# scraed/LanPaint

Measured on AMD Instinct MI355X. Metric: langevin_think_iterations_per_sec, higher is better.
Workload: dtype f32; 1 GPU; c2_sdxl: latent 1x4x128x128 per GPU, 30 sigmas x 5 think iterations, 50% box mask, stub backbone x->(0.9x,0.8x), VE/Karras schedule; rng=torch, graph=auto, mask_format=f32, mask_seen_by_kernels=bits, captured_calls=1, backbone_io=f32, replicas=1, rows_per_gpu=1, global_rows=1, latent_elements_per_gpu=65536

## Files before the change

include/lanpaint_hip.h:

```cpp
#ifndef LANPAINT_HIP_H
#define LANPAINT_HIP_H

#include <stdint.h>

#ifdef __cplusplus
extern "C" {
#endif

#define LP_ABI_VERSION 25

#define LP_API __attribute__((visibility("default")))

#define LP_OK             0
#define LP_E_INVALID     -1
#define LP_E_UNSUPPORTED -2
#define LP_E_LAUNCH      -3
#define LP_E_ALIGN       -4

#define LP_COEF_STRIDE   36
#define LP_C_SCALE        0
#define LP_C_SQRT_ABT     1
#define LP_C_OMA          2
#define LP_C_ABT          3
#define LP_C_RSIGMA       4
// ... 41 lines not shown
#define LP_FL_MASK_U8       (1u << 2)
#define LP_FL_WRITE_X0S     (1u << 3)
#define LP_FL_X0_BF16       (1u << 4)
#define LP_FL_X0_F16        (1u << 5)
#define LP_FL_XIN_BF16      (1u << 6)
#define LP_FL_XIN_F16       (1u << 7)
#define LP_FL_PER_ELEMENT   (1u << 8)
#define LP_FL_CFG_FUSED     (1u << 10)
#define LP_FL_MASK_BITS     (1u << 11)
#define LP_FL_NO_REGION_SKIP (1u << 12)
#define LP_FL_ES            (1u << 13)
#define LP_FL_ES_GATED      (1u << 14)
#define LP_FL_ES_CLOSE      (1u << 15)
#define LP_FL_ES_RING_BITS  (1u << 16)
#define LP_FL_AV            (1u << 17)
#define LP_FL_X0S_GIVEN     (1u << 9)

typedef struct lp_es_state {
    int32_t  stopped;
    int32_t  counter;
    int32_t  n_ran;
    int32_t  cur_slot;
    int32_t  anchor_slot;
    int32_t  write_slot;
    uint32_t reserved0;
    int32_t  enabled;
    int64_t  seq_base;
    int64_t  total_ran;
    double   threshold_eff;
    double   abt_val;
// ... 888 lines not shown
```

lanpaint_amd/_cabi.py:

```python
from __future__ import annotations

import ctypes as C
import os

_HERE = os.path.dirname(os.path.abspath(__file__))
LIB_NAME = "liblanpaint_hip.so"
LIB_PATH = os.path.join(_HERE, LIB_NAME)
ABI_VERSION = 25

LP_OK, LP_E_INVALID, LP_E_UNSUPPORTED, LP_E_LAUNCH, LP_E_ALIGN = 0, -1, -2, -3, -4
LP_COEF_STRIDE = 36
(LP_C_SCALE, LP_C_SQRT_ABT, LP_C_OMA, LP_C_ABT, LP_C_RSIGMA, LP_C_DTX, LP_C_DTY, LP_C_AX, LP_C_AY, LP_C_DX, LP_C_DY,
 LP_C_VALID) = range(12)
LP_C_REGION0, LP_C_REGION1, LP_C_TMODEL, LP_C_RSCALE = 12, 22, 32, 33
(LP_R_E_FULL, LP_R_K_FULL, LP_R_STD_FULL, LP_R_E_HALF, LP_R_K_HALF, LP_R_STD_HALF, LP_R_DT, LP_R_A, LP_R_CX0,
 LP_R_CXT) = range(10)

LP_PH_REPLACE, LP_PH_POST_FIRST, LP_PH_POST_STEADY, LP_PH_PRE_HALF, LP_PH_EMIT, LP_PH_COEFFS, LP_PH_SIGMA = 1, 2, 4, 8, 16, 32, 64
LP_FL_FLOW, LP_FL_MASK_DENOISE, LP_FL_MASK_U8, LP_FL_WRITE_X0S = 1, 2, 4, 8
LP_FL_X0_BF16, LP_FL_X0_F16, LP_FL_XIN_BF16, LP_FL_XIN_F16 = 16, 32, 64, 128
LP_FL_PER_ELEMENT, LP_FL_X0S_GIVEN, LP_FL_CFG_FUSED, LP_FL_MASK_BITS, LP_FL_NO_REGION_SKIP = 256, 512, 1024, 2048, 4096
LP_FL_ES, LP_FL_ES_GATED, LP_FL_ES_CLOSE, LP_FL_ES_RING_BITS, LP_FL_AV = 1 << 13, 1 << 14, 1 << 15, 1 << 16, 1 << 17
LP_TUNE_VEC1, LP_TUNE_VEC4, LP_TUNE_ES_NO_DECIDE, LP_TUNE_ES_NO_FOLD, LP_TUNE_ES_NO_ATOMICS = 1, 2, 4, 8, 16


def mask_bits_bytes(n_el: int) -> int:
    return ((int(n_el) + 63) // 64) * 8
LP_REPLACE_KNOWN, LP_REPLACE_VE, LP_REPLACE_FLOW = 0, 1, 2
LP_RNG_PHILOX, LP_RNG_TORCH = 0, 1
LP_NN_ATEN_SCALAR, LP_NN_ATEN_CPU_GENERIC_FMA, LP_NN_ATEN_CPU_GENERIC = 0, 1, 2
LP_RESHAPE_BINARIZE, LP_RESHAPE_RULE_SHIFT = 1, 8


class LpHyper(C.Structure):
    _fields_ = [("lambda_", C.c_float), ("beta", C.c_float), ("step_size", C.c_float), ("min_step_frac", C.c_float),
                ("is_flow", C.c_int32), ("one_plus_lambda", C.c_float)]

# ... 637 lines not shown
```

lanpaint_amd/buffers.py:

```python
from __future__ import annotations

import weakref

import torch

from . import _cabi
from ._util import tensor_version

class _Workspace:

    def __init__(self, like: torch.Tensor, static_io: bool = False, model_dtype=None):
        self.shape, self.device = tuple(like.shape), like.device
        self.x_t = torch.empty_like(like)
        self.C = torch.empty_like(like)
        self.coef = torch.empty((like.shape[0], _cabi.LP_COEF_STRIDE), dtype=torch.float32, device=like.device)
        self.coef_av = None
        self.av_times = None
        self.x0s = []
        self.static_io = static_io
        if static_io:
            self.x_final = torch.empty_like(like)
            self.x_in = self.x_final if model_dtype is None else torch.empty_like(like, dtype=model_dtype)

    def matches(self, like):
# ... 58 lines not shown
        return self.ring[3] if self.ring is not None else None

    def wait(self, seq, device):
        i64 = self.i64
        for _ in range(20000):
            if i64[0] >= seq:
                return
        torch.cuda.current_stream(device).synchronize()
        if i64[0] < seq:
            raise RuntimeError("early-stop mailbox was not written (expected sequence %d, found %d)" % (seq, int(i64[0])))


class _CallState:
    __slots__ = ("input_x", "xc", "shape", "n_el", "rows", "flow", "ws", "stream", "sigma", "y", "m", "m_c", "m_flag", "abt",
                 "current_times", "base_flags", "keep", "t_model", "sigma_model", "compat", "n_steps", "x_final", "x_in",
                 "xin_flag", "k0_desc", "replace_kind_static", "out", "es")


class _CapturedCall:

    def __init__(self, counter):
        self.graph = torch.cuda.CUDAGraph()
        self.counter = counter
        self.ws = None
        self.final = None
        self.ran = 0
        self.launches = 0
        self.keep = None
        self.fast = False
        self.rows, self.flow, self.hyper, self.k0_desc, self.f_desc = 0, False, None, None, None
        self.call = None
        self.raw_exec = None
        self.ident = None
        self.final_in_graph = False
        self.es = None
        self.n_steps = 0
        self.key = None
        self.tail = None
        self.model_options = None
        self.alive = True
        self.siblings = {}
        self.times_seen = ()
        self.node_table = None
        self.binding = None
        self.tail_handles = None
        self.sigma_root = None

    def __del__(self):
        sr, self.sigma_root = self.sigma_root, None
# ... 12 lines not shown
```

lanpaint_amd/capture.py:

```python
from __future__ import annotations

import ctypes
import os
import weakref

import torch

from . import _cabi
from ._util import _gc_hold, _gc_release
from .buffers import _CapturedCall, _Workspace
from .masks import _compact_mask


class GraphReplay:

    MAX_GRAPHS = 16
    AUTO_MAX_BACKBONE_HOST_US = 100.0

    def begin_call(self, x, latent_image, noise, sigma, latent_mask, current_times, model_options, seed):
        cap = self._last_cap
        if cap is None or cap.tail is None or self.model_dtype is not None or not x.is_cuda:
            return None
        self.img_dim_size = len(x.shape)
        self.latent_image, self.noise = latent_image, noise
# ... 174 lines not shown
        for seen in cap.times_seen:
            if seen[0] is ve and seen[1] is abt and seen[2] is ft:
                return True
        ok = (i[13] == ve.numel() and i[14] == abt.numel() and i[15] == ft.numel() and ve.dtype == f32 and abt.dtype == f32
              and ft.dtype == f32 and ve.is_contiguous() and abt.is_contiguous() and ft.is_contiguous())
        if ok:
            cap.times_seen = (cap.times_seen + ((ve, abt, ft),))[-2:]
        return ok

    def _hyper_key(self):
        return (self.chara_lamb, self.chara_beta, self.step_size, self.min_step_frac)

    def _override_state(self):
        d, t, o = self.__dict__, type(self), self._OWN_METHODS
        return ("langevin_dynamics" in d or t.langevin_dynamics is not o[0], "score_model" in d or t.score_model is not o[1],
                "prepare_step_size" in d or t.prepare_step_size is not o[2], self.IS_FLUX, self.IS_FLOW, self.model_dtype)

    def _graph_eligible(self, x, model_options, sigma, current_times):
        if not self.graph or self._graph_blocked or callable(self.rng) or self._noise_regenerated:
            return False
        rows = x.shape[0] if x.ndim else 1
        if any(t.numel() not in (1, rows) for t in (sigma, *current_times)):
            return False
        if self.audio_indicator is not None or self.audio_correction is not None:
            if (self.audio_indicator is None or self.current_times_audio is None
                    or any(t.numel() not in (1, rows) for t in self.current_times_audio)
                    or os.environ.get("LANPAINT_AMD_AV_TABLE", "1") == "0"):
                return False
            packed = self._indicator_pack(self.audio_indicator, x.shape)
            if packed is None or (self._es_opts is not None and not packed[2]):
                return False
# ... 50 lines not shown
            out_b = self.LanPaint(xb, sigma, latent_mask, current_times, n_steps, model_options, seed, IS_FLUX, IS_FLOW)
            same = bool(torch.equal(out_a, out_b)) and bool(torch.equal(xa, xb))
        except Exception as e:
            return give_up("checking the capture against eager launches failed (%s)" % type(e).__name__)
        if not same:
            return give_up("a replayed sigma call does not reproduce the eager one (the backbone keeps state the graph does not see)")
        self._iterations_run, _, _, self._torch_consumed, self._philox_offset = saved
        torch.cuda.set_rng_state(saved[1], dev)
        return cap

    def _call_graphed(self, x, sigma, latent_mask, current_times, n_steps, model_options, seed, IS_FLUX, IS_FLOW):
        m_c, _ = _compact_mask(latent_mask, x.shape, x.device)
        key = (tuple(x.shape), x.device.index, int(n_steps), bool(IS_FLUX), bool(IS_FLOW), self.latent_image.data_ptr(),
               latent_mask.data_ptr(), m_c.data_ptr() if m_c is not None else 0, int(sigma.numel()),
               tuple(int(t.numel()) for t in current_times), id(model_options), seed, self.rng, self._hyper_key(),
               self.model_dtype, None if self._es_opts is None else (self._es_opts["threshold"], self._es_opts["patience_eff"],
                                                                      self._es_opts["trace"] is not None),
               None if self.audio_indicator is None else (self._indicator_pack(self.audio_indicator, x.shape)[0].data_ptr(),
                                                          self.audio_correction is not None))
        cap = self._graphs.get(key)
        if cap is not None and cap.model_options is not model_options:
            del self._graphs[key]
            cap.alive = False
            cap = None
        if cap is None:
            capture = self._auto_capture if self.graph == "auto" else self._capture
            cap = capture(key, x, sigma, latent_mask, current_times, n_steps, model_options, seed, IS_FLUX, IS_FLOW)
            if cap is None:
                return self.LanPaint(x, sigma, latent_mask, current_times, n_steps, model_options, seed, IS_FLUX, IS_FLOW)
            while len(self._graphs) > self.MAX_GRAPHS:
                self._graphs.popitem(last=False)[1].alive = False
# ... 9 lines not shown
            self._last_cap = None
            return self.LanPaint(x, sigma, latent_mask, current_times, n_steps, model_options, seed, IS_FLUX, IS_FLOW)
        self._iterations_run += cap.ran
        self.last_inner_steps = cap.ran
        if fast:
            if not isinstance(model_options, dict) or "lanpaint_semantic_stop" not in model_options:
                cap.ident = (self.latent_image, latent_mask, model_options, x.shape, n_steps, seed, self.rng,
                             self.latent_image.data_ptr(), latent_mask.data_ptr(), getattr(latent_mask, "_lp_bits", None),
                             getattr(latent_mask, "_lp_u8", None), x.device, sigma.numel(), current_times[0].numel(),
                             current_times[1].numel(), current_times[2].numel(), self._override_state(), self._hyper_key())
                self._last_cap = cap
            return self._replay_fast(cap, x, sigma, current_times)
        self._last_cap = None
        st = self._prologue(x, sigma, latent_mask, current_times, n_steps, model_options, seed, IS_FLUX, IS_FLOW, ws=cap.ws,
                            ds=cap.es["ds"] if cap.es is not None else None)
        cap.graph.replay()
        if self.rng == "torch":
            gen = self._generator(x.device)
            gen.set_offset(gen.get_offset() + cap.launches)
            self._torch_consumed += cap.launches
        out = self._epilogue(st, cap.final, rng_bump=(cap.counter, cap.launches) if self.rng == "philox" else None,
                             in_graph=cap.final_in_graph)
        if cap.es is not None and st.es is not None:
            self._es_after_replay(cap, st.es["seq"], x.device)
        return out

    def _replay_fast(self, cap, x, sigma, current_times):
        lib, stream = self._lib, self._stream(x.device)
        ve, abt = current_times[0], current_times[1]
        t_src = current_times[2] if cap.flow else ve
        out = torch.empty_like(x)
        k0, f = cap.k0_desc, cap.f_desc
        k0.x, k0.noise = x.data_ptr(), self.noise.data_ptr()
        k0.t_ve, k0.t_abt, k0.t_rsig, k0.t_model = ve.data_ptr(), abt.data_ptr(), sigma.data_ptr(), t_src.data_ptr()
        if cap.final_in_graph:
            k0.io_table_val[0], k0.io_table_val[1] = k0.x, out.data_ptr()
        else:
            f.x_dst, f.out = k0.x, out.data_ptr()
        if self.rng == "torch":
            gen = self._generator(x.device)
            off = gen.get_offset()
            k0.rng_state_val[0], k0.rng_state_val[1] = off, gen.initial_seed()
            gen.set_offset(off + cap.launches)
            self._torch_consumed += cap.launches
        seq = 0
        if cap.es is not None:
            seq = k0.es_seq_base = cap.es["ds"].next_seq()
        if cap.raw_exec is not None:
            _cabi.check(lib.lp_replay_call(ctypes.byref(cap.call), stream), "lp_replay_call")
        else:
            _cabi.check(lib.lp_step(ctypes.byref(k0), stream), "lp_step")
# ... 118 lines not shown
                    cap.final_in_graph = True
        finally:
            self._capturing = None
            _gc_release()
        cap.launches = self._cap_offset
        self._es_opts = es_user
        torch.cuda.set_rng_state(rng_state, dev)
        cap.ran = self._iterations_run - it0
        self._iterations_run = it0
        cap.keep = st
        cap.rows, cap.flow = st.rows, st.flow
        cap.hyper = _cabi.LpHyper.from_buffer_copy(self._hyper)
        cap.k0_desc = st.k0_desc
        cap.f_desc = f
        cap.model_options = model_options
        cap.es, cap.n_steps = st.es, st.n_steps
        cap.fast = bool(dense_ok and st.k0_desc is not None and st.replace_kind_static and st.xc is st.input_x)
        if replace_in_graph:
            ok = cap.fast and cap.final_in_graph
            if ok:
                try:
                    cap.graph.instantiate()
                    raw_graph = int(cap.graph.raw_cuda_graph())
                    cap.raw_exec = int(cap.graph.raw_cuda_graph_exec()) or None
                    b = _cabi.LpGraphBinding()
                    ok = cap.raw_exec is not None and self._lib.lp_graph_bind_replace(
                        raw_graph, ctypes.byref(cap.k0_desc), ctypes.byref(b)) == _cabi.LP_OK
                    if ok:
                        cap.binding = b
                        tg, te = ctypes.c_void_p(), ctypes.c_void_p()
                        if self._lib.lp_graph_clone_tail(raw_graph, ctypes.byref(tg), ctypes.byref(te)) == _cabi.LP_OK:
# ... 28 lines not shown
```

lanpaint_amd/csrc/aux_kernels.hip:

```cpp
#include "lp_common.h"

namespace lp {

__global__ void lp_coeffs_kernel(lp_hyper h, const float* __restrict__ ve, int ve_stride,
                                 const float* __restrict__ abt, int abt_stride, const float* __restrict__ rs,
                                 int rs_stride, const float* __restrict__ step_ov, int step_stride,
                                 const float* __restrict__ t_model, int t_stride, int rows, float* __restrict__ table) {
    const int t = blockIdx.x * blockDim.x + threadIdx.x;
    const int r = t >> 2;
    if (r >= rows) return;
    const float abt_f = abt[static_cast<int64_t>(r) * abt_stride];
    const float ve_f = ve ? ve[static_cast<int64_t>(r) * ve_stride] : 0.0f;
    const float rs_f = rs ? rs[static_cast<int64_t>(r) * rs_stride] : 0.0f;
    const float tm_f = t_model ? t_model[static_cast<int64_t>(r) * t_stride] : 0.0f;
    const float oma = 1.0f - abt_f;
    const float step = step_ov ? step_ov[static_cast<int64_t>(r) * step_stride]
                               : h.step_size * fmaxf(oma, h.min_step_frac);
    coeffs_lane(h, abt_f, ve_f, rs_f, tm_f, step, (t >> 1) & 1, t & 1, table + static_cast<int64_t>(r) * LP_COEF_STRIDE);
}

__global__ void lp_sigma_times_kernel(const float* __restrict__ sigma, int rows, const float* __restrict__ schedule,
                                      int schedule_len, int is_flow, float* __restrict__ times,
                                      float* __restrict__ scalars, int32_t* __restrict__ seq_out, int32_t seq,
                                      const SigmaRule rule) {
// ... 26 lines not shown
    hipLaunchKernelGGL(lp_coeffs_kernel, dim3((lanes + block - 1) / block), dim3(block), 0, stream, *h, ve, ve_stride,
                       abt, abt_stride, rs, rs_stride, step_ov, step_stride, t_model, t_stride, rows, table);
    return hipGetLastError() == hipSuccess ? LP_OK : LP_E_LAUNCH;
}

template <int VEC, int BLOCK>
__global__ __launch_bounds__(256) void lp_finalize_kernel(const void* a_mask, const void* a_model_out, const float* a_y,
                                                          const float* a_x_src, const uint64_t* a_io_table, int64_t a_n_el,
                                                          uint32_t a_flags, const lp_final_desc d_arg) {
    lp_final_desc d = d_arg;
    d.mask = a_mask; d.model_out = a_model_out; d.y = a_y; d.x_src = a_x_src; d.io_table = a_io_table;
    d.n_el = a_n_el; d.flags = a_flags;
    const int64_t groups = d.n_el / VEC;
    const int dt = x0_dtype(d.flags);
    const int64_t g = static_cast<int64_t>(blockIdx.x) * BLOCK + threadIdx.x;
    float* const x_dst = d.io_table ? reinterpret_cast<float*>(d.io_table[0]) : d.x_dst;
    float* const out = d.io_table ? reinterpret_cast<float*>(d.io_table[1]) : d.out;
    if (d.io_table && d.io_table[2] == 0ull) return;
    constexpr bool RA = VEC == 4 && BLOCK == 256;
    const bool in_range = g < groups;
    if (RA || in_range) {
        const int64_t i = (in_range ? g : groups - 1) * VEC;
        float m[VEC], mo[VEC], yv[VEC], o[VEC];
        Raw<VEC> m_raw, mo_raw, un_raw;
        load_mask_raw<VEC>(d.mask, d.flags, i, m_raw);
        float xs[VEC];
        bool need_mo = true, need_y = true;
        if constexpr (RA) {
            if (x_dst) load_f32<VEC>(d.x_src, i, xs);
            if ((d.flags & LP_FL_MASK_BITS) && !(d.flags & (LP_FL_CFG_FUSED | LP_FL_NO_REGION_SKIP))) {
                const uint32_t nib = (m_raw.w[0] >> (static_cast<uint32_t>(i) & 31u)) & 0xFu;
// ... 20 lines not shown
        }
#pragma unroll
        for (int k = 0; k < VEC; ++k) o[k] = mo[k] * (1.0f - m[k]) + yv[k] * m[k];
        store_f32<VEC>(out, i, o);
        if (x_dst) store_f32<VEC>(x_dst, i, xs);
    }
    if (d.rng_bump_ptr && blockIdx.x == 0 && threadIdx.x == 0) *d.rng_bump_ptr += d.rng_bump;
}

static bool aligned(const void* p, size_t a) { return p == nullptr || (reinterpret_cast<uintptr_t>(p) % a) == 0; }

int finalize_dispatch(const lp_final_desc* dp, hipStream_t stream) {
    if (!dp) return LP_E_INVALID;
    const lp_final_desc& d = *dp;
    if (d.n_el <= 0 || !d.model_out || !d.y || !d.mask || (!d.out && !d.io_table)) return LP_E_INVALID;
    if ((d.x_dst || d.io_table) && !d.x_src) return LP_E_INVALID;
    if ((d.flags & LP_FL_CFG_FUSED) && !d.uncond) return LP_E_INVALID;
    if ((d.flags & LP_FL_MASK_BITS) && ((d.flags & (LP_FL_MASK_U8 | LP_FL_MASK_DENOISE)) || !aligned(d.mask, 4)))
        return LP_E_INVALID;
    const bool half = x0_dtype(d.flags) != DT_F32;
    const bool vec4 = (d.n_el % 4 == 0) && aligned(d.model_out, half ? 8 : 16) && aligned(d.uncond, half ? 8 : 16) &&
                      aligned(d.y, 16) &&
                      aligned(d.mask, (d.flags & (LP_FL_MASK_U8 | LP_FL_MASK_BITS)) ? 4 : 16) && aligned(d.x_src, 16) &&
                      (d.io_table ? true : (aligned(d.x_dst, 16) && aligned(d.out, 16)));
    const int vec = vec4 ? 4 : 1;
    const int64_t groups = d.n_el / vec;
    const int block = groups <= 64 * 1024 ? 64 : 256;
    const int64_t bx = (groups + block - 1) / block;
    if (bx > 0x7fffffff) return LP_E_INVALID;
#define LP_FINAL_ARGS d.mask, d.model_out, d.y, d.x_src, d.io_table, d.n_el, d.flags, d
    const dim3 grid(static_cast<unsigned>(bx));
// ... 239 lines not shown
```

lanpaint_amd/csrc/step_kernel.hip:

```cpp
#include <cstddef>

#include "lp_common.h"

#pragma clang fp contract(off)

namespace lp {

struct RegionCoef {
    float e_full, k_full, std_full, e_half, k_half, std_half, dt, a, cx0, cxt;
};

struct RowCoef {
    float scale, sqrt_abt, oma, abt, rsigma, dtx, dty, ax, ay, dx, dy, valid;
    RegionCoef reg[2];
    float rscale;
};

__device__ __forceinline__ RowCoef load_row(const float* __restrict__ coef, int row) {
    const float* c = coef + static_cast<int64_t>(row) * LP_COEF_STRIDE;
    RowCoef r;
    r.scale = c[LP_C_SCALE]; r.sqrt_abt = c[LP_C_SQRT_ABT]; r.oma = c[LP_C_OMA]; r.abt = c[LP_C_ABT];
    r.rsigma = c[LP_C_RSIGMA]; r.dtx = c[LP_C_DTX]; r.dty = c[LP_C_DTY]; r.ax = c[LP_C_AX]; r.ay = c[LP_C_AY];
    r.dx = c[LP_C_DX]; r.dy = c[LP_C_DY]; r.valid = c[LP_C_VALID];
    r.rscale = c[LP_C_RSCALE];
// ... 296 lines not shown
        row = static_cast<int>(st_base / epr) + static_cast<int>(blockIdx.y - st_round * per_round);
        const int64_t row_lo = static_cast<int64_t>(row) * epr, row_hi = row_lo + epr;
        st_lo = row_lo > st_base ? row_lo : st_base;
        st_hi = row_hi < st_base + span ? row_hi : st_base + span;
        if (row >= d.rows || st_lo >= st_hi) return;
        const int64_t i0 = st_base + static_cast<int64_t>(blockIdx.x) * kBlock, i1 = i0 + kBlock;
        bool any = false;
#pragma unroll
        for (int k = 0; k < 4; ++k) {
            const int64_t s0 = i0 + k * static_cast<int64_t>(d.rng_bg), s1 = i1 + k * static_cast<int64_t>(d.rng_bg);
            any = any || (s0 < st_hi && s1 > st_lo);
        }
        if (!any) return;
    }
    const uint32_t fl = d.flags;
    bool es_gated = false, es_idle = false;
    int es_prev = -1, es_anchor = -1, es_write = 0;
    bool es_keeper = false;
    lp_es_state es_lite;
    uint2 es_words[8];
    double es_fv[kEsSums];
    if constexpr (ES) {
        es_gated = (fl & LP_FL_ES_GATED) != 0;
        if constexpr (es_fold) {
            const int rd = (d.es_index + 1) & 1;
            const lp_es_state* sp = d.es + rd;
            if constexpr (VEC == 4) {
                const uint2* sv = reinterpret_cast<const uint2*>(sp);
#pragma unroll
                for (int k = 0; k < 8; ++k) es_words[k] = sv[k];
// ... 346 lines not shown
        if (post) {
            if constexpr (PAIR) {
                if (need_x0) load_raw_pair(d.x0, i, pair_x0, x0_raw);
                if (!(d.x0_big == d.x0 || given) && need_known) load_raw_pair(d.x0_big, i, pair_known, x0b_raw);
            } else {
                if (need_x0 && lane_x0) load_raw_w<VEC, X0W>(d.x0, x0dt, i_x0, x0_raw);
                if (!(d.x0_big == d.x0 || given) && need_known && lane_known) load_raw_w<VEC, X0W>(d.x0_big, x0dt, i_kn, x0b_raw);
            }
        }
        if constexpr (TS) {
            asm volatile("" ::"s"(rng_w0), "s"(rng_w1), "s"(d.rng_offset), "s"(d.rng_seed), "s"(d.rng_inc),
                         "s"(reinterpret_cast<uintptr_t>(d.mask)), "s"(reinterpret_cast<uintptr_t>(d.y)),
                         "s"(reinterpret_cast<uintptr_t>(d.x_in)), "s"(reinterpret_cast<uintptr_t>(d.x0s)),
                         "s"(HARD ? uintptr_t(0) : reinterpret_cast<uintptr_t>(d.corr_el)), "s"(d.lambda),
                         "s"(d.one_plus_lambda), "s"(d.cfg_scale), "s"(d.cfg_scale_big));
        }
        if constexpr (SMALL) load_mask_raw<VEC>(d.mask, mfl, i, m_raw);
        const bool has_corr = (TS && HARD) ? false : (d.corr_el != nullptr && !given);
        const bool host_post = HOT ? false : d.xi_post != nullptr, host_pre = HOT ? false : d.xi_pre != nullptr;
        const bool need_rng = (post && !host_post) || ((ph & LP_PH_PRE_HALF) && !host_pre);
        if (post) {
            if (!given && need_known && lane_known) load_f32<VEC>(d.y, i_kn, yv);
            if (host_post) load_f32<VEC>(d.xi_post, i, xi_a);
            if (has_corr) load_f32<VEC>(d.corr_el, i, corr);
        }
        if ((ph & LP_PH_PRE_HALF) && host_pre) load_f32<VEC>(d.xi_pre, i, xi_b);
        float x0p[VEC], anc[VEC], rg[VEC], es_b0[VEC], es_b1[VEC], es_b2[VEC];
        constexpr bool RING_BITS_ONLY = ES != 0 && HARD && PH != 0;
        const bool ring_bits = RING_BITS_ONLY || (fl & LP_FL_ES_RING_BITS) != 0;
        uint32_t rg_raw = 0u;
// ... 27 lines not shown
                }
                if constexpr (!(es_fold && VEC == 4)) {
                    load_ring();
                }
            }
        }

        if constexpr (!SMALL) {
            if (need_rng && d.rng_offset_ptr) {
                rng_w0 = d.rng_offset_ptr[0];
                rng_w1 = d.rng_offset_ptr[1];
                rng_have = true;
            }
        }
        if constexpr (!TS) {
        if (d.io_table_out && el_bx == 0 && blockIdx.y == 0 && threadIdx.x == 0) {
            d.io_table_out[0] = d.io_table_val[0];
            d.io_table_out[1] = d.io_table_val[1];
            if (d.io_valid) d.io_table_out[2] = 1ull;
        }
        }
        if constexpr (PH == 0 || (PH & LP_PH_REPLACE) != 0) {
            if (d.es_reset && d.es && el_bx == 0 && blockIdx.y == 0) {
                if (d.es_partials) {
                    for (int k = threadIdx.x; k < kEsSets * kEsSlots * 8; k += kBlock) d.es_partials[k] = 0.0;
                }
                if (threadIdx.x == 0) es_reset_state(d, fold_coeffs);
            }
        }
        if constexpr (TBL) {
            float abt_f, ve_f, rs_f, tm_f;
// ... 67 lines not shown
                    }
                } else {
#pragma unroll
                for (int k = 0; k < VEC; ++k) {
                    float za, zb;
                    const uint64_t e = static_cast<uint64_t>(elem_index(i, k));
                    if (key_uniform) normal_pair_key<PH != 0>(static_cast<uint32_t>(e), static_cast<uint32_t>(seq), key0, za, zb);
                    else normal_pair(e, seq, seed, za, zb);
                    if (!host_post) xi_a[k] = za;
                    if (!host_pre) xi_b[k] = zb;
                }
                }
            }
        }

        if constexpr (TS) {
            __builtin_amdgcn_sched_barrier(0);
            if constexpr (X0W == 2) {
                uint16_t h = static_cast<uint16_t>(x0_raw.w[0]);
                asm volatile("" : "+v"(h) : "v"(xi_a[0]));
                x0_raw.w[0] = h;
            } else {
                asm volatile("" : "+v"(x0_raw.w[0]) : "v"(xi_a[0]));
            }
        }
        if constexpr (ES == 2 && VEC == 4) {
            if (post) {
                if (es_prev >= 0) load_f32<VEC>(es_prev == 0 ? d.es_x0s[0] : es_prev == 1 ? d.es_x0s[1] : d.es_x0s[2], i, x0p);
                load_ring();
            }
// ... 273 lines not shown
                for (int k = 0; k < VEC; ++k) {
                    const float ha = half_valid(xt[k], cv[k], xi_b[k], rc.reg[0]), hb = half_valid(xt[k], cv[k], xi_b[k], rc.reg[1]);
                    xe[k] = m[k] == 1.0f ? hb : ha;
                }
            } else {
#pragma unroll
                for (int k = 0; k < VEC; ++k) xe[k] = half_step(xt[k], cv[k], xi_b[k], k);
            }
            if (!(ES && es_gated)) {
#pragma unroll
                for (int k = 0; k < VEC; ++k) xt[k] = xe[k];
            }
        }

        LP_CLK(5)
        if (post && live) store_f32<VEC>(d.C, i, cv);
        if ((ph & kTouchXt) && live) store_f32<VEC>(d.x_t, i, xt);
        if constexpr (ES) {
            if (es_gated && (ph & LP_PH_PRE_HALF) && live) store_f32<VEC>(d.es_xte, i, xe);
            if (es_fold && es_idle) load_f32<VEC>(d.x_t, i, xe);
        }

        if (ph & LP_PH_EMIT) {
            float xo[VEC];
            if constexpr (VEC == 4 && !PER_EL && PH != 0) {
                const float sc = rc.scale;
                if (flow) {
                    float y;
                    if constexpr (ES != 0 || (RNG == 1 && !ST)) {
                        y = 1.0f / sc;
                        asm volatile("" : "+v"(y));
                    } else {
// ... 10 lines not shown
                for (int k = 0; k < VEC; ++k) {
                    float sc;
                    if constexpr (PER_EL) {
                        sc = flow ? (sqrtf(abt_e[k]) + sqrtf(1.0f - abt_e[k])) : sqrtf(1.0f + ve_e[k] * ve_e[k]);
                    } else {
                        sc = row_scale_of(k);
                    }
                    xo[k] = flow ? xe[k] / sc : xe[k] * sc;
                }
            }
            if constexpr (PAIR) {
                if (xindt != DT_F32) store_half_pair(d.x_in, xindt, i, xo);
                else store_any<VEC>(d.x_in, xindt, i, xo);
            } else {
                if (active) store_any<VEC>(d.x_in, xindt, i, xo);
            }
        }
    }

    LP_CLK(6)
    if constexpr (!ES) {
        LP_CLK_FLUSH
    }
    if constexpr (ES) {
        if (es_idle || !post) return;
        __shared__ float es_part[4][kEsSums];
        const int lane = threadIdx.x & (kWave - 1), wave = threadIdx.x / kWave;
        if (!es_zero_wave) wave_sum_dpp(es_p);
        if (lane == kWave - 1) {
#pragma unroll
// ... 110 lines not shown
                return rt ? plan_es<VEC, MODE_HARD, S | P | E, 4, 1>(d, p) : plan_es<VEC, MODE_HARD, S | P | E, 4, 0>(d, p);
            if (d.phases == (F | P | E))
                return rt ? plan_es<VEC, MODE_HARD, F | P | E, 4, 1>(d, p) : plan_es<VEC, MODE_HARD, F | P | E, 4, 0>(d, p);
        }
        return hard ? plan_es<VEC, MODE_HARD, 0>(d, p) : plan_es<VEC, MODE_ROW, 0>(d, p);
    }
    if (d.flags & LP_FL_MASK_U8) return plan_kernel<VEC, MODE_ROW, 0>(d, p);
    if (d.phases == (R | E | LP_PH_COEFFS))
        return hard ? plan_kernel<VEC, MODE_HARD, R | E | LP_PH_COEFFS>(d, p) : plan_kernel<VEC, MODE_ROW, R | E | LP_PH_COEFFS>(d, p);
    if (d.phases == (R | E | LP_PH_COEFFS | LP_PH_SIGMA))
        return plan_kernel<VEC, MODE_HARD, R | E | LP_PH_COEFFS | LP_PH_SIGMA>(d, p);
    const bool rng_torch = d.rng_kind == LP_RNG_TORCH;
    const bool strided = VEC == 4 && rng_torch && !d.xi_post && !d.xi_pre && d.n_el > static_cast<int64_t>(d.rng_bg) &&
                         (d.rng_bg % kBlock) == 0 &&
                         (d.rows == 1 || d.el_per_row >= 2 * static_cast<int64_t>(d.rng_bg)) && st_segments(d) != 0;
    const bool ts_rare = VEC == 1 && rng_torch && (d.n_el > static_cast<int64_t>(d.rng_bg) || d.io_table_out != nullptr);
    if (!pair_ok || rare || ts_rare) return hard ? plan_kernel<VEC, MODE_HARD, 0>(d, p) : plan_kernel<VEC, MODE_ROW, 0>(d, p);
    if (hard) {
        switch (d.phases) {
            case S | P | E: return plan_hot<VEC, MODE_HARD, S | P | E>(d, strided, x0_half, rng_torch, p);
            case F | P | E: return plan_hot<VEC, MODE_HARD, F | P | E>(d, strided, x0_half, rng_torch, p);
            case S | E: return plan_hot<VEC, MODE_HARD, S | E>(d, strided, x0_half, rng_torch, p);
            default: return plan_kernel<VEC, MODE_HARD, 0>(d, p);
        }
    }
    switch (d.phases) {
        case S | P | E: return plan_hot<VEC, MODE_ROW, S | P | E>(d, strided, x0_half, rng_torch, p);
        case F | P | E: return plan_hot<VEC, MODE_ROW, F | P | E>(d, strided, x0_half, rng_torch, p);
        case S | E: return plan_hot<VEC, MODE_ROW, S | E>(d, strided, x0_half, rng_torch, p);
        default: return plan_kernel<VEC, MODE_ROW, 0>(d, p);
    }
// ... 18 lines not shown
        if (!d.av_bits || !aligned(d.av_bits, 4) || !d.coef || (d.flags & LP_FL_PER_ELEMENT) || (ph & (LP_PH_COEFFS | LP_PH_SIGMA)) ||
            !(d.av_frac >= 0.0f && d.av_frac <= 1.0f))
            return LP_E_INVALID;
    }
    if (d.rng_kind != LP_RNG_PHILOX && d.rng_kind != LP_RNG_TORCH) return LP_E_INVALID;
    if (d.rng_kind == LP_RNG_TORCH && (d.rng_bg == 0 || (d.rng_inc & 3u) || d.rng_inc == 0)) return LP_E_INVALID;
    if (ph & LP_PH_COEFFS) {
        if ((ph & ~LP_PH_SIGMA) != (LP_PH_REPLACE | LP_PH_EMIT | LP_PH_COEFFS) || (d.flags & LP_FL_PER_ELEMENT)) return LP_E_INVALID;
        if (!d.coef_out) return LP_E_INVALID;
        if (!(ph & LP_PH_SIGMA)) {
            if (!d.t_abt || (!(d.flags & LP_FL_FLOW) && !d.t_ve)) return LP_E_INVALID;
            if (d.replace_kind != LP_REPLACE_KNOWN && !d.t_rsig) return LP_E_INVALID;
        }
    }
    if ((ph & LP_PH_POST_FIRST) && (ph & LP_PH_POST_STEADY)) return LP_E_INVALID;
    if ((ph & LP_PH_REPLACE) && (ph & (kPost | LP_PH_PRE_HALF))) return LP_E_INVALID;
    const bool per_el = d.flags & LP_FL_PER_ELEMENT;
    if (!per_el && !d.coef && !(ph & LP_PH_COEFFS)) return LP_E_INVALID;
    if (per_el && (!d.abt_el || (!(d.flags & LP_FL_FLOW) && !d.ve_el))) return LP_E_INVALID;
    if (ph & LP_PH_REPLACE) {
        if (!d.x) return LP_E_INVALID;
        if (d.replace_kind == LP_REPLACE_KNOWN) {
            if (!d.known) return LP_E_INVALID;
        } else if (d.replace_kind == LP_REPLACE_VE || d.replace_kind == LP_REPLACE_FLOW) {
            if (!d.noise || !d.y) return LP_E_INVALID;
            if (per_el && !d.rsig_el) return LP_E_INVALID;
        } else {
            return LP_E_INVALID;
        }
    }
// ... 107 lines not shown
    Timer* timer = static_cast<Timer*>(timer_handle);
    StepPlan p;
    const int rc = plan_step(*dp, &p, timer != nullptr);
    return rc == LP_OK ? enqueue(p, *dp, stream, timer) : rc;
}

int replace_node_update(const lp_step_desc* dp, hipGraphExec_t exec, const lp_graph_binding* b) {
    if (!dp || !exec || !b || !b->node || !b->func) return LP_E_INVALID;
    const lp_step_desc& d = *dp;
    if (!(d.phases & LP_PH_REPLACE) || d.xi_post || d.xi_pre || (d.flags & LP_FL_X0S_GIVEN)) return LP_E_INVALID;
    StepPlan p;
    const int rc = plan_step(d, &p);
    if (rc != LP_OK) return rc;
    if (!plan_is_node(p, b->func, dim3(b->grid[0], b->grid[1], b->grid[2]), dim3(b->block[0], b->block[1], b->block[2])))
        return LP_E_INVALID;
    StepArgs a;
    pack_step_args(p, d, &a);
    hipKernelNodeParams np{};
    np.func = const_cast<void*>(p.kernel);
    np.gridDim = p.grid;
    np.blockDim = dim3(kBlock);
    np.sharedMemBytes = b->shared_bytes;
    np.kernelParams = a.ptr;
    np.extra = nullptr;
    return hipGraphExecKernelNodeSetParams(exec, static_cast<hipGraphNode_t>(b->node), &np) == hipSuccess ? LP_OK : LP_E_LAUNCH;
}

int timer_create(void** out) {
    if (!out) return LP_E_INVALID;
    Timer* t = new Timer();
// ... 29 lines not shown
```

lanpaint_amd/engine.py:

```python
from __future__ import annotations

import ctypes
import os
import weakref
from collections import OrderedDict
from time import perf_counter

import torch

from . import _cabi
from ._cabi import (LP_FL_ES, LP_FL_ES_GATED, LP_FL_ES_CLOSE, LP_FL_CFG_FUSED, LP_FL_FLOW, LP_FL_MASK_BITS, LP_FL_MASK_U8, LP_FL_XIN_BF16,
                    LP_FL_XIN_F16, LP_FL_PER_ELEMENT, LP_FL_WRITE_X0S, LP_FL_X0_BF16, LP_FL_X0_F16, LP_FL_X0S_GIVEN, LP_PH_EMIT,
                    LP_PH_POST_FIRST, LP_PH_POST_STEADY, LP_PH_PRE_HALF, LP_PH_REPLACE, LP_REPLACE_FLOW, LP_REPLACE_KNOWN,
                    LP_REPLACE_VE)
from ._util import _as_f32c, _noise_scaling_kind, aten_randn_policy, raw_stream, tensor_version
from .buffers import _CallState, _Workspace
from .earlystop import HostStopper, StopOptions
from .masks import _compact_mask, pack_indicator, pack_mask, refresh_packed_mask
from .types import FusedCFGHeads


class EngineCore:

    def __init__(self, Model, NSteps, Friction, Lambda, Beta, StepSize, IS_FLUX=False, IS_FLOW=False,
                 EarlyStopThreshold=0.0, EarlyStopPatience=1, EarlyStopHook=None, MinStepFrac=0.0,
                 *, rng=None, philox_seed=None, graph=None, model_dtype=None, early_stop_group=None):
# ... 36 lines not shown
        self._ws = None
        self._desc = _cabi.LpStepDesc()
        self._fdesc = _cabi.LpFinalDesc()
        self._hyper = _cabi.LpHyper()
        self._noise_check = None
        self.assume_static_noise = False
        self.auto_pack_mask = os.environ.get("LANPAINT_AMD_AUTO_PACK", "1") != "0"
        self._mask_seen = None
        self._noise_regenerated = False
        self._iterations_run = 0
        self.last_inner_steps = 0
        self.early_stop_group = early_stop_group
        self._ds = None
        self._es_opts = None
        self._es_pending = None

    @property
    def iterations_run(self):
        self._es_resolve()
        return self._iterations_run

    @iterations_run.setter
    def iterations_run(self, v):
        self._iterations_run = v

    def _indicator_pack(self, indicator, shape):
        c = getattr(self, "_av_pack", None)
        if c is None or c[0] is not indicator or c[1] != tuple(shape):
            c = self._av_pack = (indicator, tuple(shape), pack_indicator(indicator, shape))
        return c[2]
# ... 377 lines not shown
                known = _as_f32c(ms.noise_scaling(self.add_none_dims(replace_sigma), nz, y))
                keep.append(known)
                d.replace_kind, d.known = LP_REPLACE_KNOWN, known.data_ptr()
            elif kind == "ve":
                d.replace_kind = LP_REPLACE_VE
            else:
                d.replace_kind, d.noise_scale = LP_REPLACE_FLOW, ns
        else:
            d.replace_kind, d.noise_scale = LP_REPLACE_FLOW, float(getattr(ms, "noise_scale", 1.0))

        st.compat = self._overridden("langevin_dynamics") or self._overridden("score_model") or \
            self._overridden("prepare_step_size")
        if n_steps > 0 and float(self.step_size) <= 0.0 and not st.compat:
            n_steps = 0
        st.n_steps = n_steps

        if ws.static_io:
            st.x_final, st.x_in = ws.x_final, ws.x_in
        else:
            st.x_final = torch.empty_like(xc)
            st.x_in = st.x_final if self.model_dtype is None else torch.empty_like(xc, dtype=self.model_dtype)
        st.xin_flag = 0 if self.model_dtype is None else (LP_FL_XIN_BF16 if self.model_dtype == torch.bfloat16 else LP_FL_XIN_F16)

        d.x = xc.data_ptr()
        d.xi_post = d.xi_pre = None
        d.rng_offset_ptr = None
        d.rng_seed = int(self.philox_seed if self.philox_seed is not None else (seed or 0)) & 0xFFFFFFFFFFFFFFFF
        d.rng_state_out = None
        if ws.static_io and self.rng == "torch" and not per_el:
            gen = self._generator(xc.device)
# ... 35 lines not shown
            d.x_in = st.x_final.data_ptr()
            return 0
        d.x_in = st.x_in.data_ptr()
        return st.xin_flag

    def _think_and_final_model(self, st, model_options, seed):
        d, ws, shape, base_flags, n_steps, stream = self._desc, st.ws, st.shape, st.base_flags, st.n_steps, st.stream
        d.n_el, d.el_per_row, d.rows = st.n_el, st.n_el // st.rows, st.rows
        stopper = None
        if self._capturing is None and st.es is None:
            stopper = HostStopper.from_options(
                StopOptions.parse(model_options, self.early_stop_threshold, self.early_stop_patience, self.early_stop_hook),
                st.m, st.abt)
            if stopper is not None and self.early_stop_group is not None:
                stopper.sums.reduce_group = self.early_stop_group
        ran = 0
        if st.compat:
            ran = self._loop_compat(ws, shape, st.m, st.y, st.abt, st.current_times, n_steps, model_options, seed, stopper)
            d.phases = LP_PH_EMIT
            d.flags = base_flags | self._emit(st, True)
            self._launch_step(stream)
        elif st.es is not None:
            ran = self._loop_es(st, n_steps, model_options, seed)
        elif stopper is not None:
            ran = self._loop_unfused(st, n_steps, model_options, seed, stopper)
        else:
            auto = self._auto if (self.graph == "auto" and self._capturing is None) else None
            bb_s = 0.0
            for i in range(n_steps):
                last = i == n_steps - 1
                if auto is not None:
                    t_bb = perf_counter()
                    output = self.inner_model(st.x_in, st.t_model, model_options=model_options, seed=seed)
                    bb_s += perf_counter() - t_bb
                else:
                    output = self.inner_model(st.x_in, st.t_model, model_options=model_options, seed=seed)
                alive = self._set_model_output(d, output, base_flags | self._emit(st, last), shape)
                d.phases = (LP_PH_POST_FIRST if i == 0 else LP_PH_POST_STEADY) | (0 if last else LP_PH_PRE_HALF) | LP_PH_EMIT
                self._set_xi(d, ws.x_t, want_pre=not last)
                self._launch_step(stream)
                del alive
            ran = n_steps
            if auto is not None and n_steps > 0:
                auto[1] += 1
                auto[2] = min(auto[2], bb_s / n_steps)
        self._iterations_run += ran
        self.last_inner_steps = ran
        x_model = st.x_final if self.model_dtype is None else st.x_final.to(self.model_dtype)
        return self.inner_model(x_model, st.sigma_model, model_options=model_options, seed=seed)

    def _fill_final_desc(self, f, st, final, out):
        shape = st.shape
        converted = []

        def dense(t):
            t0 = t
            if t.shape != shape:
                t = t.expand(shape)
            if t.dtype not in (torch.float32, torch.bfloat16, torch.float16):
                t = t.float()
            t = t if t.is_contiguous() else t.contiguous()
            if t is not t0:
                converted.append(t)
            return t

        uncond = None
        if isinstance(final, FusedCFGHeads) and final._heads is None and final.cond.dtype == final.uncond.dtype:
            out_model, uncond = dense(final.cond), dense(final.uncond)
            f.cfg_scale = final.scale
        else:
            out_model = dense(self.unpack_model_output(final)[0])
        f.n_el = st.n_el
        f.flags = (LP_FL_X0_BF16 if out_model.dtype == torch.bfloat16 else
                   LP_FL_X0_F16 if out_model.dtype == torch.float16 else 0) | (LP_FL_CFG_FUSED if uncond is not None else 0) \
            | st.m_flag
        f.uncond = uncond.data_ptr() if uncond is not None else None
        f.model_out, f.y = out_model.data_ptr(), st.y.data_ptr()
        f.mask = st.m_c.data_ptr() if st.m_c is not None else st.m.data_ptr()
        f.x_src, f.x_dst, f.out = st.x_final.data_ptr(), st.xc.data_ptr(), out.data_ptr()
        f.rng_bump_ptr, f.rng_bump, f.io_table = None, 0, None
        self._final_alive = (out_model, uncond)
        return not converted

    def _epilogue(self, st, final, rng_bump=None, in_graph=False):
        f, xc = self._fdesc, st.xc
        out = st.out if st.out is not None else torch.empty_like(xc)
        if not in_graph:
            self._fill_final_desc(f, st, final, out)
            if rng_bump is not None:
                f.rng_bump_ptr, f.rng_bump = rng_bump[0].data_ptr(), int(rng_bump[1])
            _cabi.check(self._lib.lp_finalize(ctypes.byref(f), st.stream), "lp_finalize")
        if xc is not st.input_x:
            st.input_x.copy_(xc)
        return out if out.dtype == st.input_x.dtype else out.to(st.input_x.dtype)
# ... 35 lines not shown
```

Before: 125,800 think-iterations/s.

## Fuse final x writeback into last Langevin step, skipping finalize copy

Adds a CLOSE flag so the last think iteration writes the final latent straight into the caller's x (or an io-table target in graph mode). That step then skips its C and x_t stores, and the finalize kernel no longer copies x_final to xc. The aim is to cut memory traffic and one copy pass per call. In exchange it adds new kernel template paths, io-table alignment checks and extra graph-capture key state, which could raise register pressure or add edge-case correctness risk.

```diff
diff --git a/include/lanpaint_hip.h b/include/lanpaint_hip.h
--- a/include/lanpaint_hip.h
+++ b/include/lanpaint_hip.h
@@ -79,6 +79,7 @@
 #define LP_FL_ES_CLOSE      (1u << 15)
 #define LP_FL_ES_RING_BITS  (1u << 16)
 #define LP_FL_AV            (1u << 17)
+#define LP_FL_CLOSE         (1u << 18)
 #define LP_FL_X0S_GIVEN     (1u << 9)
 
 typedef struct lp_es_state {
diff --git a/lanpaint_amd/_cabi.py b/lanpaint_amd/_cabi.py
--- a/lanpaint_amd/_cabi.py
+++ b/lanpaint_amd/_cabi.py
@@ -21,6 +21,7 @@
 LP_FL_X0_BF16, LP_FL_X0_F16, LP_FL_XIN_BF16, LP_FL_XIN_F16 = 16, 32, 64, 128
 LP_FL_PER_ELEMENT, LP_FL_X0S_GIVEN, LP_FL_CFG_FUSED, LP_FL_MASK_BITS, LP_FL_NO_REGION_SKIP = 256, 512, 1024, 2048, 4096
 LP_FL_ES, LP_FL_ES_GATED, LP_FL_ES_CLOSE, LP_FL_ES_RING_BITS, LP_FL_AV = 1 << 13, 1 << 14, 1 << 15, 1 << 16, 1 << 17
+LP_FL_CLOSE = 1 << 18
 LP_TUNE_VEC1, LP_TUNE_VEC4, LP_TUNE_ES_NO_DECIDE, LP_TUNE_ES_NO_FOLD, LP_TUNE_ES_NO_ATOMICS = 1, 2, 4, 8, 16
 
 
diff --git a/lanpaint_amd/buffers.py b/lanpaint_amd/buffers.py
--- a/lanpaint_amd/buffers.py
+++ b/lanpaint_amd/buffers.py
@@ -96,7 +96,7 @@
 class _CallState:
     __slots__ = ("input_x", "xc", "shape", "n_el", "rows", "flow", "ws", "stream", "sigma", "y", "m", "m_c", "m_flag", "abt",
                  "current_times", "base_flags", "keep", "t_model", "sigma_model", "compat", "n_steps", "x_final", "x_in",
-                 "xin_flag", "k0_desc", "replace_kind_static", "out", "es")
+                 "xin_flag", "k0_desc", "replace_kind_static", "out", "es", "close")
 
 
 class _CapturedCall:
@@ -115,6 +115,7 @@
         self.raw_exec = None
         self.ident = None
         self.final_in_graph = False
+        self.close = False
         self.es = None
         self.n_steps = 0
         self.key = None
diff --git a/lanpaint_amd/capture.py b/lanpaint_amd/capture.py
--- a/lanpaint_amd/capture.py
+++ b/lanpaint_amd/capture.py
@@ -212,7 +212,8 @@
     def _override_state(self):
         d, t, o = self.__dict__, type(self), self._OWN_METHODS
         return ("langevin_dynamics" in d or t.langevin_dynamics is not o[0], "score_model" in d or t.score_model is not o[1],
-                "prepare_step_size" in d or t.prepare_step_size is not o[2], self.IS_FLUX, self.IS_FLOW, self.model_dtype)
+                "prepare_step_size" in d or t.prepare_step_size is not o[2], self.IS_FLUX, self.IS_FLOW, self.model_dtype,
+                self.close_launch)
 
     def _graph_eligible(self, x, model_options, sigma, current_times):
         if not self.graph or self._graph_blocked or callable(self.rng) or self._noise_regenerated:
@@ -293,7 +294,7 @@
         key = (tuple(x.shape), x.device.index, int(n_steps), bool(IS_FLUX), bool(IS_FLOW), self.latent_image.data_ptr(),
                latent_mask.data_ptr(), m_c.data_ptr() if m_c is not None else 0, int(sigma.numel()),
                tuple(int(t.numel()) for t in current_times), id(model_options), seed, self.rng, self._hyper_key(),
-               self.model_dtype, None if self._es_opts is None else (self._es_opts["threshold"], self._es_opts["patience_eff"],
+               self.model_dtype, self.close_launch, None if self._es_opts is None else (self._es_opts["threshold"], self._es_opts["patience_eff"],
                                                                       self._es_opts["trace"] is not None),
                None if self.audio_indicator is None else (self._indicator_pack(self.audio_indicator, x.shape)[0].data_ptr(),
                                                           self.audio_correction is not None))
@@ -333,6 +334,7 @@
         self._last_cap = None
         st = self._prologue(x, sigma, latent_mask, current_times, n_steps, model_options, seed, IS_FLUX, IS_FLOW, ws=cap.ws,
                             ds=cap.es["ds"] if cap.es is not None else None)
+        st.close = cap.close
         cap.graph.replay()
         if self.rng == "torch":
             gen = self._generator(x.device)
@@ -354,6 +356,9 @@
         k0.t_ve, k0.t_abt, k0.t_rsig, k0.t_model = ve.data_ptr(), abt.data_ptr(), sigma.data_ptr(), t_src.data_ptr()
         if cap.final_in_graph:
             k0.io_table_val[0], k0.io_table_val[1] = k0.x, out.data_ptr()
+        elif cap.close:
+            k0.io_table_val[0], k0.io_table_val[1] = k0.x, out.data_ptr()
+            f.out = out.data_ptr()
         else:
             f.x_dst, f.out = k0.x, out.data_ptr()
         if self.rng == "torch":
@@ -502,7 +507,7 @@
         cap.k0_desc = st.k0_desc
         cap.f_desc = f
         cap.model_options = model_options
-        cap.es, cap.n_steps = st.es, st.n_steps
+        cap.es, cap.n_steps, cap.close = st.es, st.n_steps, st.close
         cap.fast = bool(dense_ok and st.k0_desc is not None and st.replace_kind_static and st.xc is st.input_x)
         if replace_in_graph:
             ok = cap.fast and cap.final_in_graph
diff --git a/lanpaint_amd/csrc/aux_kernels.hip b/lanpaint_amd/csrc/aux_kernels.hip
--- a/lanpaint_amd/csrc/aux_kernels.hip
+++ b/lanpaint_amd/csrc/aux_kernels.hip
@@ -64,7 +64,7 @@
     const int64_t groups = d.n_el / VEC;
     const int dt = x0_dtype(d.flags);
     const int64_t g = static_cast<int64_t>(blockIdx.x) * BLOCK + threadIdx.x;
-    float* const x_dst = d.io_table ? reinterpret_cast<float*>(d.io_table[0]) : d.x_dst;
+    float* const x_dst = !d.x_src ? nullptr : d.io_table ? reinterpret_cast<float*>(d.io_table[0]) : d.x_dst;
     float* const out = d.io_table ? reinterpret_cast<float*>(d.io_table[1]) : d.out;
     if (d.io_table && d.io_table[2] == 0ull) return;
     constexpr bool RA = VEC == 4 && BLOCK == 256;
@@ -115,7 +115,7 @@
     if (!dp) return LP_E_INVALID;
     const lp_final_desc& d = *dp;
     if (d.n_el <= 0 || !d.model_out || !d.y || !d.mask || (!d.out && !d.io_table)) return LP_E_INVALID;
-    if ((d.x_dst || d.io_table) && !d.x_src) return LP_E_INVALID;
+    if (d.x_dst && !d.x_src) return LP_E_INVALID;
     if ((d.flags & LP_FL_CFG_FUSED) && !d.uncond) return LP_E_INVALID;
     if ((d.flags & LP_FL_MASK_BITS) && ((d.flags & (LP_FL_MASK_U8 | LP_FL_MASK_DENOISE)) || !aligned(d.mask, 4)))
         return LP_E_INVALID;
diff --git a/lanpaint_amd/csrc/step_kernel.hip b/lanpaint_amd/csrc/step_kernel.hip
--- a/lanpaint_amd/csrc/step_kernel.hip
+++ b/lanpaint_amd/csrc/step_kernel.hip
@@ -334,6 +334,8 @@
         if (!any) return;
     }
     const uint32_t fl = d.flags;
+    constexpr bool CAN_CLOSE = ES == 0 && !PER_EL && (PH == 0 || PH == (LP_PH_POST_STEADY | LP_PH_EMIT));
+    const bool close = CAN_CLOSE && (fl & LP_FL_CLOSE) != 0;
     bool es_gated = false, es_idle = false;
     int es_prev = -1, es_anchor = -1, es_write = 0;
     bool es_keeper = false;
@@ -710,6 +712,19 @@
                          "s"(reinterpret_cast<uintptr_t>(d.x_in)), "s"(reinterpret_cast<uintptr_t>(d.x0s)),
                          "s"(HARD ? uintptr_t(0) : reinterpret_cast<uintptr_t>(d.corr_el)), "s"(d.lambda),
                          "s"(d.one_plus_lambda), "s"(d.cfg_scale), "s"(d.cfg_scale_big));
+            if constexpr (CAN_CLOSE) asm volatile("" ::"s"(reinterpret_cast<uintptr_t>(d.io_table_out)), "s"(reinterpret_cast<uintptr_t>(d.x)));
+        }
+        uint64_t cl_w0 = 0, cl_w2 = 0;
+        if constexpr (CAN_CLOSE) {
+            typedef const __attribute__((address_space(4))) uint64_t* table_words;
+            const bool cl_tbl = close && d.io_table_out != nullptr;
+            if constexpr (PH != 0) {
+                const table_words tw = (table_words)(cl_tbl ? d.io_table_out : reinterpret_cast<const uint64_t*>(d.coef));
+                cl_w0 = tw[0]; cl_w2 = tw[2];
+            } else if (cl_tbl) {
+                const table_words tw = (table_words)d.io_table_out;
+                cl_w0 = tw[0]; cl_w2 = tw[2];
+            }
         }
         if constexpr (SMALL) load_mask_raw<VEC>(d.mask, mfl, i, m_raw);
         const bool has_corr = (TS && HARD) ? false : (d.corr_el != nullptr && !given);
@@ -767,7 +782,7 @@
             }
         }
         if constexpr (!TS) {
-        if (d.io_table_out && el_bx == 0 && blockIdx.y == 0 && threadIdx.x == 0) {
+        if (d.io_table_out && !close && el_bx == 0 && blockIdx.y == 0 && threadIdx.x == 0) {
             d.io_table_out[0] = d.io_table_val[0];
             d.io_table_out[1] = d.io_table_val[1];
             if (d.io_valid) d.io_table_out[2] = 1ull;
@@ -865,6 +880,7 @@
             }
         }
 
+        if constexpr (CAN_CLOSE && PH != 0) asm volatile("" ::"s"(cl_w0), "s"(cl_w2));
         if constexpr (TS) {
             __builtin_amdgcn_sched_barrier(0);
             if constexpr (X0W == 2) {
@@ -1168,8 +1184,8 @@
         }
 
         LP_CLK(5)
-        if (post && live) store_f32<VEC>(d.C, i, cv);
-        if ((ph & kTouchXt) && live) store_f32<VEC>(d.x_t, i, xt);
+        if (post && live && !close) store_f32<VEC>(d.C, i, cv);
+        if ((ph & kTouchXt) && live && !close) store_f32<VEC>(d.x_t, i, xt);
         if constexpr (ES) {
             if (es_gated && (ph & LP_PH_PRE_HALF) && live) store_f32<VEC>(d.es_xte, i, xe);
             if (es_fold && es_idle) load_f32<VEC>(d.x_t, i, xe);
@@ -1210,6 +1226,10 @@
                 else store_any<VEC>(d.x_in, xindt, i, xo);
             } else {
                 if (active) store_any<VEC>(d.x_in, xindt, i, xo);
+            }
+            if (close) {
+                float* const x_out = d.io_table_out ? (cl_w2 != 0ull ? reinterpret_cast<float*>(cl_w0) : nullptr) : const_cast<float*>(d.x);
+                if (x_out && active) store_f32<VEC>(x_out, i, xo);
             }
         }
     }
@@ -1350,7 +1370,8 @@
     const bool strided = VEC == 4 && rng_torch && !d.xi_post && !d.xi_pre && d.n_el > static_cast<int64_t>(d.rng_bg) &&
                          (d.rng_bg % kBlock) == 0 &&
                          (d.rows == 1 || d.el_per_row >= 2 * static_cast<int64_t>(d.rng_bg)) && st_segments(d) != 0;
-    const bool ts_rare = VEC == 1 && rng_torch && (d.n_el > static_cast<int64_t>(d.rng_bg) || d.io_table_out != nullptr);
+    const bool ts_rare = VEC == 1 && rng_torch && (d.n_el > static_cast<int64_t>(d.rng_bg) ||
+                                                   (d.io_table_out != nullptr && !(d.flags & LP_FL_CLOSE)));
     if (!pair_ok || rare || ts_rare) return hard ? plan_kernel<VEC, MODE_HARD, 0>(d, p) : plan_kernel<VEC, MODE_ROW, 0>(d, p);
     if (hard) {
         switch (d.phases) {
@@ -1399,6 +1420,11 @@
         }
     }
     if ((ph & LP_PH_POST_FIRST) && (ph & LP_PH_POST_STEADY)) return LP_E_INVALID;
+    if (d.flags & LP_FL_CLOSE) {
+        if (!(ph & kPost) || !(ph & LP_PH_EMIT) || (ph & ~(kPost | LP_PH_EMIT))) return LP_E_UNSUPPORTED;
+        if (d.flags & (LP_FL_ES | LP_FL_PER_ELEMENT | LP_FL_AV)) return LP_E_UNSUPPORTED;
+        if (!d.io_table_out && !d.x) return LP_E_INVALID;
+    }
     if ((ph & LP_PH_REPLACE) && (ph & (kPost | LP_PH_PRE_HALF))) return LP_E_INVALID;
     const bool per_el = d.flags & LP_FL_PER_ELEMENT;
     if (!per_el && !d.coef && !(ph & LP_PH_COEFFS)) return LP_E_INVALID;
@@ -1536,6 +1562,7 @@
     if (rc != LP_OK) return rc;
     if (!plan_is_node(p, b->func, dim3(b->grid[0], b->grid[1], b->grid[2]), dim3(b->block[0], b->block[1], b->block[2])))
         return LP_E_INVALID;
+    if (p.vec == 4 && d.io_table_out && ((d.io_table_val[0] | d.io_table_val[1]) & 15ull)) return LP_E_ALIGN;
     StepArgs a;
     pack_step_args(p, d, &a);
     hipKernelNodeParams np{};
diff --git a/lanpaint_amd/engine.py b/lanpaint_amd/engine.py
--- a/lanpaint_amd/engine.py
+++ b/lanpaint_amd/engine.py
@@ -9,7 +9,7 @@
 import torch
 
 from . import _cabi
-from ._cabi import (LP_FL_ES, LP_FL_ES_GATED, LP_FL_ES_CLOSE, LP_FL_CFG_FUSED, LP_FL_FLOW, LP_FL_MASK_BITS, LP_FL_MASK_U8, LP_FL_XIN_BF16,
+from ._cabi import (LP_FL_CLOSE, LP_FL_ES, LP_FL_ES_GATED, LP_FL_ES_CLOSE, LP_FL_CFG_FUSED, LP_FL_FLOW, LP_FL_MASK_BITS, LP_FL_MASK_U8, LP_FL_XIN_BF16,
                     LP_FL_XIN_F16, LP_FL_PER_ELEMENT, LP_FL_WRITE_X0S, LP_FL_X0_BF16, LP_FL_X0_F16, LP_FL_X0S_GIVEN, LP_PH_EMIT,
                     LP_PH_POST_FIRST, LP_PH_POST_STEADY, LP_PH_PRE_HALF, LP_PH_REPLACE, LP_REPLACE_FLOW, LP_REPLACE_KNOWN,
                     LP_REPLACE_VE)
@@ -76,6 +76,7 @@
         self._ds = None
         self._es_opts = None
         self._es_pending = None
+        self.close_launch = os.environ.get("LANPAINT_AMD_CLOSE_LAUNCH", "1") != "0"
 
     @property
     def iterations_run(self):
@@ -483,6 +484,7 @@
         if n_steps > 0 and float(self.step_size) <= 0.0 and not st.compat:
             n_steps = 0
         st.n_steps = n_steps
+        st.close = bool(self.close_launch and n_steps >= 1 and not per_el and av is None and corr is None and not st.compat)
 
         if ws.static_io:
             st.x_final, st.x_in = ws.x_final, ws.x_in
@@ -548,6 +550,7 @@
                 st.m, st.abt)
             if stopper is not None and self.early_stop_group is not None:
                 stopper.sums.reduce_group = self.early_stop_group
+        st.close = close = bool(st.close and not st.compat and st.es is None and stopper is None)
         ran = 0
         if st.compat:
             ran = self._loop_compat(ws, shape, st.m, st.y, st.abt, st.current_times, n_steps, model_options, seed, stopper)
@@ -569,10 +572,17 @@
                     bb_s += perf_counter() - t_bb
                 else:
                     output = self.inner_model(st.x_in, st.t_model, model_options=model_options, seed=seed)
-                alive = self._set_model_output(d, output, base_flags | self._emit(st, last), shape)
+                if last and close:
+                    emit = self._emit(st, self.model_dtype is None) | LP_FL_CLOSE
+                    d.x = st.xc.data_ptr()
+                    d.io_table_out = self._rng_state(st.xc.device).data_ptr() + 16 if ws.static_io else None
+                else:
+                    emit = self._emit(st, last)
+                alive = self._set_model_output(d, output, base_flags | emit, shape)
                 d.phases = (LP_PH_POST_FIRST if i == 0 else LP_PH_POST_STEADY) | (0 if last else LP_PH_PRE_HALF) | LP_PH_EMIT
                 self._set_xi(d, ws.x_t, want_pre=not last)
                 self._launch_step(stream)
+                d.io_table_out = None
                 del alive
             ran = n_steps
             if auto is not None and n_steps > 0:
@@ -580,7 +590,10 @@
                 auto[2] = min(auto[2], bb_s / n_steps)
         self._iterations_run += ran
         self.last_inner_steps = ran
-        x_model = st.x_final if self.model_dtype is None else st.x_final.to(self.model_dtype)
+        if self.model_dtype is None:
+            x_model = st.x_final
+        else:
+            x_model = st.x_in if close else st.x_final.to(self.model_dtype)
         return self.inner_model(x_model, st.sigma_model, model_options=model_options, seed=seed)
 
     def _fill_final_desc(self, f, st, final, out):
@@ -611,7 +624,10 @@
         f.uncond = uncond.data_ptr() if uncond is not None else None
         f.model_out, f.y = out_model.data_ptr(), st.y.data_ptr()
         f.mask = st.m_c.data_ptr() if st.m_c is not None else st.m.data_ptr()
-        f.x_src, f.x_dst, f.out = st.x_final.data_ptr(), st.xc.data_ptr(), out.data_ptr()
+        if st.close:
+            f.x_src, f.x_dst, f.out = None, None, out.data_ptr()
+        else:
+            f.x_src, f.x_dst, f.out = st.x_final.data_ptr(), st.xc.data_ptr(), out.data_ptr()
         f.rng_bump_ptr, f.rng_bump, f.io_table = None, 0, None
         self._final_alive = (out_model, uncond)
         return not converted
```

New measurement: 125,800 think-iterations/s (median of 3 runs). No clear change (+0.0%).
